# bobwan1995/cliora

Measured on AMD Instinct MI355X. Metric: sentences/sec (inside+outside fwd+bwd), len-20 d=400 bsz=64, higher is better.
Workload: dtype f32 (compose GEMMs: 3x bf16 MFMA per product, fp32 accumulate)

## Files before the change

### cliora_amd/csrc/api_mlp.hip

```cpp
#include "api_mlp_launch.hpp"
#include "ragged_kernels.hpp"
#include "resident_kernels.hpp"
#include "vl_kernels.hpp"

static bool wavefront_pays(const Plan& p, int env) {
    if (p.L <= 2 || env == 0) return false;
    if (env >= 1) return true;
    const double row_floats_per_level = (double)(p.R_in + p.R_out) / (2.0 * (p.L - 1)) * p.Dp;
    return row_floats_per_level >= 100e3;
}

static bool merged_pays(const Plan& p) {
    if (p.arch != 0 || p.L <= 2) return false;
    if (g_cliora_wavefront != 2 && !(g_cliora_wavefront < 0 && wavefront_pays(p, -1))) return false;
    for (size_t e = 0; e < (size_t)2 * p.L; ++e) {
        const int sp = p.level_geom[e * PLEVEL_INTS + 6];
        if (p.level_geom[e * PLEVEL_INTS + 1] > 0 && !project2_parts_ok(sp)) return false;
    }
    return true;
}

static size_t resident_lds_bytes(const Plan& p) {
    return ((size_t)(p.share ? 7 : 8) * p.Dp * p.Dp + (size_t)RES_WAVES * RES_SCR) * sizeof(float);
}
// ... 496 lines not shown
    const float *x_span, *obj_span, *drop_mask, *inside_h, *IS, *outside_h, *OS;
    const float *d_inside_h, *d_inside_s, *d_outside_h, *d_outside_s;
    float *ws, *wb, *d_x_span, *d_obj_span;
    int ran_outside;
    hipStream_t st;

    const Plan& p = plan->p;
    const FwdLayout& f = p.fwd;
    const BwdLayout& bw = p.bwd;
    const Dev dv = dev_views(p);
    const int B = p.B, L = p.L, D = p.D, Dp = p.Dp, C = p.C, nb = p.nblk, ldpi = nb * Dp;
    const bool vl = p.R > 0, padded = D != Dp;
    const bool compress = P && P->root_mat;
    const BwdSchedule schedule = compress ? BwdSchedule::OutsideThenInside
                               : resident_pays(plan, vl, compress) ? BwdSchedule::Resident : BwdSchedule::Wavefront;
    const bool resident = schedule == BwdSchedule::Resident;
    const bool two_streams = schedule == BwdSchedule::Wavefront && ran_outside && wavefront_pays(p, g_cliora_wavefront);
    const hipStream_t sb = two_streams ? plan->side : st, sw = plan->side2;
    const float *IH = padded ? ws + f.ihp : inside_h, *OH = padded ? ws + f.ohp : outside_h;
    const float *X = padded ? ws + f.xp : x_span, *OBJ = vl ? (padded ? ws + f.objp : obj_span) : nullptr;
    const float *IHn = vl ? ws + f.att_u : IH, *nrmIn = vl ? ws + f.att_nrmu : ws + f.nrmi;
    float *VH = wb + bw.vh, *dG = wb + bw.dg, *dStot = wb + bw.dstot, *VHo = wb + bw.vh_o, *dGo = wb + bw.dg_o, *dStoto = wb + bw.dstot_o;
    float *DA = wb + bw.da, *DS = wb + bw.ds, *dPI = wb + bw.dpi, *dPO = wb + bw.dpo, *dU = wb + bw.du;
    float *DZ = wb + bw.dz, *Xp = wb + bw.x, *DPP = wb + bw.dpp, *DPB = wb + bw.dpb;
    const float *Sp = ws + f.sp, *Pp = ws + f.pp, *PI = ws + f.pi;
    const uint32_t* YM = reinterpret_cast<const uint32_t*>(ws + f.ymask);
    const bool fuse_dnorm = schedule == BwdSchedule::Wavefront;
    const int gemm3_shape = split_bf16() ? bwd_gemm3_env() : 0;
    const bool tiled = pair_tiles_ok(Dp) && !resident;
    float *sibPL = p.share ? wb + bw.sib_pl : dPI + (size_t)3 * Dp, *sibQL = p.share ? wb + bw.sib_ql : dPI + (size_t)4 * Dp;
    const int ldsib = p.share ? Dp : ldpi;
    const int sib_split = two_streams ? (L * 2) / 5 : 0;

    bool sibling_runs(int s_level) const { return s_level >= 0 && s_level <= p.L - 1 && ran_outside && s_level < sib_split; }

    template <class EP>
    int project_bwd(hipStream_t s, const float* WT, const float* WTfrag, const float* W3s, int K, int ncell, const LevelRowsA& rows, EP ep) const {
        if (gemm3_shape > 0) return launch_rows_direct3x(s, W3s, K, p.Dp, ncell, rows, ep, gemm3_shape);
        return launch_rows_direct(s, WT, WTfrag, IMG_FRAG_F32, K, p.Dp, ncell, rows, ep);
    }
    int project_bwd_level(hipStream_t s, bool outside, const LevelArgs& g, bool fused_norm) const {
        const int ldp = outside ? Dp : ldpi, ncell = B * g.Lc;
        const float *WT = ws + (outside ? f.w1roT : f.wcatT), *WTfrag = ws + (outside ? f.w1roT3 : f.wcatT3), *W3s = ws + (outside ? f.w1roT3s : f.wcatT3s);
        const LevelRowsA rows{outside ? dPO : dPI, ldp, p.C, g.off, g.Lc};
        float* vh = outside ? VHo : VH;
        if (fused_norm)
            return project_bwd(s, WT, WTfrag, W3s, ldp, ncell, rows,
                               NormBwdLevelE{outside ? dGo : dG, vh, outside ? OH : IH, ws + (outside ? f.nrmo : f.nrmi),
                                             wb + (outside ? bw.dots_o : bw.dots), Dp, p.C, g.off, g.Lc, p.normalize});
        return project_bwd(s, WT, WTfrag, W3s, ldp, ncell, rows, StoreLevelE{vh, Dp, p.C, g.off, g.Lc, nullptr, 1});
    }

    int outside_bwd_step(int level, hipEvent_t done) const {
        const LevelArgs g = level_args(p, level, true);
        const int ncell = B * g.Lc;
        const bool fused_norm = fuse_dnorm && level >= 1 && level <= L - 2;
        hipLaunchKernelGGL(cell_gather_bwd_out, dim3(ncell), dim3(256), 0, sb, g, p.D, d_outside_h,
                           level == L - 1 ? nullptr : d_outside_s, dv.use[ROLE_OUTB], DA, DS, PI, ldpi, p.blk_qlo, dPO, VHo, dStoto,
                           OH, ws + f.po, fused_norm ? wb + bw.dots_o : nullptr);
        LAUNCHOK("cell_gather_bwd_out");
        if (level >= 1) OKR(project_bwd_level(sb, true, g, fused_norm));
        if (level == L - 1) {
            if (compress) {
                hipLaunchKernelGGL(cell_dnorm, dim3(cells_grid(ncell)), dim3(256), 0, sb, g, VHo, OH, ws + f.nrmo, p.normalize, dGo);
                LAUNCHOK("cell_dnorm(root)");
                return CLIORA_OK;
            }
            LAUNCH_SIGNALLING(done, root_bwd, dim3(1), dim3(ROOT_WAVES * 64), 0, sb, B, C, Dp, VHo, OH, ws + f.nrmo, p.normalize, wb + bw.groot);
            LAUNCHOK("root_bwd");
            return CLIORA_OK;
        }
        if (!fused_norm) {
            hipLaunchKernelGGL(cell_dnorm, dim3(cells_grid(ncell)), dim3(256), 0, sb, g, VHo, OH, ws + f.nrmo, p.normalize, dGo);
            LAUNCHOK("cell_dnorm(out)");
        }
        {
            ProfScope ps(CLIORA_KCLASS_COMPOSE_BWD, sb);
            OKR(launch_level_compose_bwd(sb, ws + f.w2oT, ws + f.w2oT3, f.S3, Dp, f.ct3, f.ncb3, pair_level(p, level, true), dGo, YM, Pp,
                                         PI + (size_t)p.blk_plo * Dp, ldpi, ws + f.po, Dp, ws + f.b2o, DA, DZ, Xp, DPP, DPB, tiled));
        }
        const int s_level = L - 2 - level;
        const bool sib_last = sibling_runs(s_level);
        LAUNCH_SIGNALLING(sib_last ? nullptr : done, cell_dsoftmax, dim3(cells_grid(ncell)), dim3(256), 0, sb, g, f.ncb3, DPP, DPB, Sp, Pp, OS, dStoto, DS);
        LAUNCHOK("cell_dsoftmax(out)");
        if (sib_last) {
            const LevelArgs gi = level_args(p, s_level, false);
            LAUNCH_SIGNALLING(done, cell_gather_bwd_sib, dim3(B * gi.Lc), dim3(256), 0, sb, gi, dv.use[ROLE_OUTA], DA, DS, OH, sibPL, sibQL, ldsib, wb + bw.sib_s);
            LAUNCHOK("cell_gather_bwd_sib");
        }
        return CLIORA_OK;
    }

    WgradPlacement wgrad_placement() const {
        static const int ksplit_env = [] { const char* e = getenv("CLIORA_WGRAD_SPLIT_LEVEL"); return e ? atoi(e) : -1; }();
        const bool wcat_split_path = split_bf16() && tn_pairs_strided_ok(p.Dp);
        const bool sw_beside = plan->side2_beside;
        WgradPlacement w{};
        w.ksplit = ksplit_env >= 0 ? ksplit_env : !sw_beside ? 0
                 : wcat_split_path ? std::max(1, std::min(2 * L / 5, L - 1)) : std::min(2, L - 1);
        w.tail_cells = p.C;
        static const int early_env = [] { const char* e = getenv("CLIORA_WGRAD_EARLY_STEP"); return e ? atoi(e) : -2; }();
        const int early_auto = L >= 16 && sw_beside ? L / 2 + 1 : -1;
        const int early_pick = early_env == -2 ? early_auto : early_env;
        w.J_early = (p.share && ran_outside && schedule == BwdSchedule::Wavefront && early_pick >= 0 && early_pick <= L - 3) ? early_pick : -1;
        const int early2_pick = L >= 28 ? (w.J_early + L) / 2 : -1;
        w.J_early2 = (w.J_early >= 0 && early2_pick > w.J_early && early2_pick <= L - 3) ? early2_pick : -1;
        return w;
    }
    int wcat_grad(hipStream_t s_, int off, int hi, int accumulate) const {
        if (tn_pairs_strided_ok(Dp) && (long long)B * hi >= 512 && (long long)B * hi < (1LL << 22)) {
            return launch_tn_level_block(s_, dPI, ldpi, IH, B, C, off, hi, Dp, wb + bw.slab2, bw.slab_floats, wb + bw.gwcat, wb + bw.gbcat, accumulate,
                                         std::max(8, (180 / (3 * nb)) / 4 * 4), nb);
        }
        return launch_tn(s_, B * hi, ldpi, Dp, Dp, LevelRowsA{dPI, ldpi, C, off, hi}, LevelRowsA{IH, Dp, C, off, hi}, wb + bw.slab2,
                         bw.slab_floats, wb + bw.gwcat, wb + bw.gbcat, accumulate);
    }
    int pair_rows_early(WgradPlacement& w, int j) const {
        const bool first = j == w.J_early;
        const bool second = tiled && w.J_early >= 0 && j == w.J_early2;
        if (!first && !second) return CLIORA_OK;
// ... 96 lines not shown
        const size_t DD = (size_t)Dp * Dp;
        if (vl && d_obj_span && padded) add_copy(t, d_obj_span, D, B * p.R, D, wb + bw.dobjp, Dp, B * p.R, D, 0, 0, 0);
        if (G->leaf_w) add_copy(t, G->leaf_w, D, D, D, wb + bw.gwl, Dp, D, D, 0, 0, 0);
        if (G->leaf_b) add_copy(t, G->leaf_b, D, 1, D, wb + bw.gbl, Dp, 1, D, 0, 0, 0);
        if (G->root_h && !compress) add_copy(t, G->root_h, D, 1, D, wb + bw.groot, Dp, 1, D, 0, 0, 0);
        if (G->root_mat && compress) add_copy(t, G->root_mat, D, D, D, wb + bw.groot_mat, Dp, D, D, 0, 0, 1);
        const bool early = p.share && w.J_early >= 0;
        if (G->in_w1) {
            add_copy(t, G->in_w1, 2 * D, D, D, wb + bw.gwcat, Dp, D, D, 0, 0, 0);
            add_copy(t, G->in_w1 + D, 2 * D, D, D, wb + bw.gwcat + DD, Dp, D, D, 0, 0, 0, p.share ? wb + bw.gw1ro : nullptr, Dp, D, D, 0, 0, 0);
        }
        if (G->in_b1) add_copy(t, G->in_b1, D, 1, D, wb + bw.gbcat, Dp, 1, D, 0, 0, 0);
        if (G->in_mat) add_copy(t, G->in_mat, D, D, D, wb + bw.gwcat + 2 * DD, Dp, D, D, 0, 0, 1);
        if (G->in_w2) add_copy(t, G->in_w2, D, D, D, wb + bw.gw2i, Dp, D, D, 0, 0, 0, early ? wb + bw.gw2o : nullptr, Dp, D, D, 0, 0, 0);
        if (G->in_b2) add_copy(t, G->in_b2, D, 1, D, wb + bw.gb2i, Dp, 1, D, 0, 0, 0, early ? wb + bw.gb2o : nullptr, Dp, 1, D, 0, 0, 0);
        if (!p.share) {
            if (G->out_w1) {
                add_copy(t, G->out_w1, 2 * D, D, D, wb + bw.gwcat + 3 * DD, Dp, D, D, 0, 0, 0);
                add_copy(t, G->out_w1 + D, 2 * D, D, D, wb + bw.gw1ro, Dp, D, D, 0, 0, 0);
            }
            if (G->out_b1) add_copy(t, G->out_b1, D, 1, D, wb + bw.gbcat + 3 * Dp, Dp, 1, D, 0, 0, 0);
            if (G->out_mat) add_copy(t, G->out_mat, D, D, D, wb + bw.gwcat + 4 * DD, Dp, D, D, 0, 0, 1);
            if (G->out_w2) add_copy(t, G->out_w2, D, D, D, wb + bw.gw2o, Dp, D, D, 0, 0, 0);
            if (G->out_b2) add_copy(t, G->out_b2, D, 1, D, wb + bw.gb2o, Dp, 1, D, 0, 0, 0);
        }
        return run_copies(st, t);
    }

    int inside_bwd_step(WgradPlacement& w, int level) const {
        hipStream_t sa = st;
        const LevelArgs g = level_args(p, level, false);
        const int ncell = B * g.Lc;
        const bool fused_norm = fuse_dnorm && p.share && !vl && level >= 1 && level <= L - 2;
        hipLaunchKernelGGL(cell_gather_bwd_in, dim3(ncell), dim3(256), 0, sa, g, p.D, d_inside_h,
                           level == 0 ? nullptr : d_inside_s, dv.use[ROLE_INA], dv.use[ROLE_INB], dv.use[ROLE_OUTA],
                           !ran_outside ? 0 : (level < sib_split ? 1 : 2),
                           sibPL, sibQL, ldsib, wb + bw.sib_s, DA, DS, PI, ldpi, p.share, IH, OH, dPI, VH, dStot,
                           ws + f.bcat, fused_norm ? wb + bw.dots : nullptr);
        LAUNCHOK("cell_gather_bwd_in");
        if (level == 0) {
            HIPOK(hipEventRecord(plan->ev_fork[2], sa));
            w.dpi_done_recorded = true;
        }
        if (level <= L - 2) OKR(project_bwd_level(sa, false, g, fused_norm));
        else if (compress && ran_outside)
            OKR(launch_rows_direct(sa, ws + f.rootwT, PROJ_IMG(f.rootwT3), Dp, Dp, ncell, LevelRowsA{dGo, Dp, C, g.off, g.Lc},
                                   StoreLevelE{VH, Dp, C, g.off, g.Lc, nullptr, 1}));
        if (vl) {
            with_regions(p.R, [&](auto NR) {
                hipLaunchKernelGGL(cell_attend_bwd<decltype(NR)::value>, dim3(ncell), dim3(256), 0, sa, g, VH, IH, ws + f.nrmi, p.normalize, OBJ, p.R,
                                   drop_mask, ws + f.att_pk, wb + bw.dctx, wb + bw.pmo, wb + bw.dsc, IHn, nrmIn, level >= 1 ? dG : (float*)nullptr);
            });
            LAUNCHOK("cell_attend_bwd");
        }
        if (level == w.ksplit && level >= 1) {
            HIPOK(hipEventRecord(plan->ev_fork[2], sa));
            HIPOK(hipStreamWaitEvent(sw, plan->ev_fork[2], 0));
            OKR(wcat_grad(sw, g.off, w.tail_cells - g.off, w.tail_cells < C));
            w.tail_cells = g.off;
        }
        if (level == 0) return CLIORA_OK;
        if (!fused_norm && !vl) {
            hipLaunchKernelGGL(cell_dnorm, dim3(cells_grid(ncell)), dim3(256), 0, sa, g, VH, IHn, nrmIn, p.normalize, dG);
            LAUNCHOK("cell_dnorm(in)");
        }
        {
            ProfScope ps(CLIORA_KCLASS_COMPOSE_BWD, sa);
            OKR(launch_level_compose_bwd(sa, ws + f.w2iT, ws + f.w2iT3, f.S3, Dp, f.ct3, f.ncb3, pair_level(p, level, false), dG, YM, Pp, PI, ldpi,
                                         PI + Dp, ldpi, ws + f.b2i, DA, DZ, Xp, DPP, DPB, tiled));
        }
        hipLaunchKernelGGL(cell_dsoftmax, dim3(cells_grid(ncell)), dim3(256), 0, sa, g, f.ncb3, DPP, DPB, Sp, Pp, IS, dStot, DS);
        LAUNCHOK("cell_dsoftmax(in)");
        if (level == 1 && two_streams) HIPOK(hipEventRecord(plan->ev_join[2], sa));
        return CLIORA_OK;
    }

    int backward_wavefront(WgradPlacement& w) const {
        for (int j = 0; j <= L - 1; ++j) {
            if (ran_outside) OKR(outside_bwd_step(j, two_streams ? plan->ev_level[j] : nullptr));
            if (two_streams && j >= 1) HIPOK(hipStreamWaitEvent(st, plan->ev_level[j - 1], 0));
            OKR(inside_bwd_step(w, L - 1 - j));
            OKR(pair_rows_early(w, j));
        }
        return CLIORA_OK;
    }

    int backward_outside_then_inside(WgradPlacement& w) const {
        for (int j = 0; j <= L - 1 && ran_outside; ++j) OKR(outside_bwd_step(j, nullptr));
        for (int j = 0; j <= L - 1; ++j) OKR(inside_bwd_step(w, L - 1 - j));
        if (ran_outside)
            return launch_tn(st, p.B, Dp, Dp, Dp, LevelRowsA{dGo, Dp, C, C - 1, 1}, LevelRowsA{IH, Dp, C, C - 1, 1}, wb + bw.slab, bw.slab_floats,
                             wb + bw.groot_mat, (float*)nullptr);
        HIPOK(hipMemsetAsync(wb + bw.groot_mat, 0, (size_t)Dp * Dp * sizeof(float), st));
        return CLIORA_OK;
    }

    int backward_resident() const {
        ResArgs a = resident_args(plan, ws, const_cast<float*>(IH), const_cast<float*>(OH), const_cast<float*>(IS), const_cast<float*>(OS), ran_outside);
        a.dIH = d_inside_h; a.dIS = d_inside_s; a.dOH = d_outside_h; a.dOS = d_outside_s;
        a.VHo = VHo; a.dPI = dPI; a.dPO = dPO; a.DA = DA; a.DS = DS; a.DZ = DZ; a.Xrows = Xp; a.dU = dU; a.dX = d_x_span;
        a.trace = res_trace() ? reinterpret_cast<unsigned long long*>(plan->trace_words) : nullptr;
        OKR(cliora_ensure_max_lds((const void*)resident_bwd));
        {
            ProfScope ps(CLIORA_KCLASS_COMPOSE_BWD, st);
            hipLaunchKernelGGL(resident_bwd, dim3(std::min(p.B, std::max(1, plan->ncu))), dim3(RES_THREADS), resident_lds_bytes(p), st, a);
// ... 67 lines not shown
```

### cliora_amd/csrc/api_mlp_launch.hpp

```cpp
#pragma once
#include "api_common.hpp"
#include "level_kernels.hpp"

template <class F>
static auto with_regions(int R, F&& f) {
    return R <= 36 ? f(Int<9>{}) : f(Int<16>{});
}

template <class F>
static int with_compose_shape(int ct, int Dp, F&& f) {
    auto mode = [&](auto CT, auto K16) { return split_bf16() ? f(CT, K16, Bool<false>{}) : f(CT, K16, Bool<true>{}); };
    if (ct == 5 && Dp == 400) return mode(Int<5>{}, Int<25>{});
    return with_int<5, 4, 2, 1>(ct, [&](auto CT) { return mode(CT, Int<0>{}); });
}
static int compose_image_stride(int S3, int Dp) { return split_bf16() ? S3 : Dp; }

template <class F>
static int with_parts(int SP, F&& f) {
    return with_int<1, 2, 3, 4>(SP, f);
}
static bool project2_parts_ok(int SP) { return SP == 1 || SP == 2 || SP == 4; }
template <class F>
static int with_parts2(int SP, F&& f) {
    return with_int<1, 2, 4>(SP, f);
// ... 15 lines not shown
        constexpr bool f32 = decltype(F32)::value;
        OKR(cliora_ensure_max_lds((const void*)level_compose_fwd<ct_, k16, f32>));
        hipLaunchKernelGGL((level_compose_fwd<ct_, k16, f32>), dim3(sg.gx, ncb), dim3(512), compose_lds_bytes(ct_, S, true), st, sg.Wimg, S, Dp, sg.lv,
                           sg.PA, sg.lda, sg.PB, sg.ldb, sg.bias, Pp, sg.TG, sg.SP, sg.ntask, sg.HP, hp_stride, Dp, ymask, Y);
        LAUNCHOK("level_compose_fwd");
        return CLIORA_OK;
    });
}

static int launch_level_compose2(hipStream_t st, const ComposeSeg& a, const ComposeSeg& b, int S3, int Dp, int ct, int ncb, const float* Pp,
                                 size_t hp_stride, uint32_t* ymask, float* Y) {
    if (a.gx + b.gx <= 0) return CLIORA_OK;
    const int S = compose_image_stride(S3, Dp);
    const int gx = xcd_pad(a.gx + b.gx);
    return with_compose_shape(ct, Dp, [&](auto CT, auto K16, auto F32) {
        constexpr int ct_ = decltype(CT)::value, k16 = decltype(K16)::value;
        constexpr bool f32 = decltype(F32)::value;
        if constexpr (k16 == 25 && !f32) {
            const size_t lds_dual = compose_lds_bytes(ct_, S, true) + (size_t)ct_ * 16 * sizeof(float);
            OKR(cliora_ensure_max_lds((const void*)level_compose_fwd2<ct_, k16, f32, 2>));
            hipLaunchKernelGGL((level_compose_fwd2<ct_, k16, f32, 2>), dim3(gx, ncb), dim3(512), lds_dual, st, a, b, S, Dp, Pp, hp_stride, Dp, ymask, Y);
            LAUNCHOK("level_compose_fwd2(dual)");
        } else {
            OKR(cliora_ensure_max_lds((const void*)level_compose_fwd2<ct_, k16, f32>));
            hipLaunchKernelGGL((level_compose_fwd2<ct_, k16, f32>), dim3(gx, ncb), dim3(512), compose_lds_bytes(ct_, S, true), st, a, b, S, Dp, Pp, hp_stride, Dp, ymask, Y);
            LAUNCHOK("level_compose_fwd2");
        }
        return CLIORA_OK;
    });
}

static int launch_level_compose_bwd(hipStream_t st, const float* WT, const float* WTimg, int S3, int Dp, int ct, int ncb, const PairLevel& lv,
                                    const float* dG, const uint32_t* ymask, const float* Pp, const float* PA, int lda, const float* PB,
                                    int ldb, const float* b2, float* DA, float* DZ, float* X, float* DPP, float* DPB, bool tiled = false, int cus = 256) {
    if (lv.N <= 0 || lv.ncell <= 0) return CLIORA_OK;
    const uint32_t* I = reinterpret_cast<const uint32_t*>(split_bf16() ? WTimg : WT);
    const int S = compose_image_stride(S3, Dp), K = Dp;
    auto launch = [&](auto CT, auto K16, auto F32, auto TILED) {
        constexpr int ct_ = decltype(CT)::value, k16 = decltype(K16)::value;
        constexpr bool f32 = decltype(F32)::value, tiled_ = decltype(TILED)::value;
        OKR(cliora_ensure_max_lds((const void*)level_compose_bwd<ct_, k16, f32, tiled_>));
        const int gx = ws_grid((lv.ncell + 15) / 16 * lv.N, ncb, 8, cus);
        hipLaunchKernelGGL((level_compose_bwd<ct_, k16, f32, tiled_>), dim3(gx, ncb), dim3(512), compose_lds_bytes(ct_, S, false) + (size_t)((K + 31) / 32 * 32) * sizeof(float), st, I, S, K, lv, dG, ymask,
                           Pp, PA, lda, PB, ldb, b2, K, DA, DZ, X, DPP, DPB);
        LAUNCHOK("level_compose_bwd");
        return CLIORA_OK;
    };
    if (tiled) {
        if (!split_bf16() || ct != 5 || Dp != 400) return fail(CLIORA_EINVAL, "tiled pair-row operands: d = 400 in split-bf16 mode only");
        return launch(Int<5>{}, Int<25>{}, Bool<false>{}, Bool<true>{});
    }
    return with_compose_shape(ct, Dp, [&](auto CT, auto K16, auto F32) { return launch(CT, K16, F32, Bool<false>{}); });
}

static int launch_level_project(hipStream_t st, int SP, const ProjSeg& q, hipEvent_t stop, bool lng) {
    const int nt = q.ntc, nrg = (q.ncell + 15) / 16;
    const int nrgp = xcd_pad(nrg);
    auto launch = [&](auto CT, auto SP_, auto LONG) {
        const int ncb = nt / decltype(CT)::value;
        LAUNCH_SIGNALLING(stop, (level_project<decltype(CT)::value, decltype(SP_)::value, decltype(LONG)::value>), dim3(q.sc.nscore + nrgp * ncb),
                          dim3(256), 0, st, q.Wfrag, q.K, nrg, nrgp, ncb, q.ncell, q.Lc, q.C, q.off, q.HP, q.hp_stride, q.normalize, q.bias, q.P,
                          q.ldp, q.H, q.nrm, q.sc);
        LAUNCHOK("level_project");
        return CLIORA_OK;
    };
    const bool wide = nt % 5 == 0 && nrg * (nt / 5) >= KSPLIT_MIN_BLOCKS;
    return with_long(lng, [&](auto LONG) {
        return with_parts(SP, [&](auto SP_) { return wide ? launch(Int<5>{}, SP_, LONG) : launch(Int<1>{}, SP_, LONG); });
    });
}

static int launch_level_project2(hipStream_t st, int SP0, int SP1, const ProjSeg& a, const ProjSeg& b, bool lng) {
    if (!project2_parts_ok(SP0) || !project2_parts_ok(SP1)) return fail(CLIORA_EINVAL, "level_project2: parts per level must be 1, 2 or 4");
    const int n = a.sc.nscore + b.sc.nscore + a.nproj + b.nproj + a.nfin + b.nfin;
    if (n <= 0) return CLIORA_OK;
    return with_long(lng, [&](auto LONG) {
        return with_parts2(SP0, [&](auto S0) {
// ... 9 lines not shown
```

### cliora_amd/csrc/chart_kernels.hpp

```cpp
#pragma once
#include <hip/hip_runtime.h>
#include <stdint.h>

#include "gemm_kernels.hpp"

namespace cliora {

constexpr float UNIT_EPS = 1e-8f;

__device__ __forceinline__ int cell_of_block(int bid, int B, int Lc) {
    const int n8 = (B >> 3) * 8 * Lc;
    if (bid >= n8) return bid;
    const int x = bid & 7, q = bid >> 3;
    const int bb = q / Lc, p = q - bb * Lc;
    return (bb * 8 + x) * Lc + p;
}

struct LevelArgs {
    int B, C, Dp, Lc, N, off;
    int rowbase;
};

__device__ __forceinline__ float4 ld4(const float* p) { return *reinterpret_cast<const float4*>(p); }
__device__ __forceinline__ void st4(float* p, float4 v) { *reinterpret_cast<float4*>(p) = v; }
// ... 77 lines not shown
            if (a1) v += f4dot(ld4(qa + 4 * (lane + 64)), ld4(hb + 4 * (lane + 64)));
            d[j] = v;
        }
#pragma unroll
        for (int j = 0; j < 4; ++j) {
            const float s = wave_sum(d[j]) + SA[ar[j]] + SB[br[j]];
            if (lane == 0 && n0 + 4 * j < g.N) sh_s[n0 + 4 * j] = s;
        }
    }
    __syncthreads();
    if (wave != 0) return;
    const float my_s = lane < g.N ? sh_s[lane] : -INFINITY;
    const float m = wave_max(my_s);
    const float e = lane < g.N ? expf(my_s - m) : 0.f;
    const float pn = e / wave_sum(e);
    if (lane < g.N) { Sp[row0 + lane] = my_s; Pp[row0 + lane] = pn; }
    const float st = wave_sum(lane < g.N ? pn * my_s : 0.f);
    if (lane == 0) Sout[(size_t)b * g.C + g.off + p] = st;
}



struct UseTab { const int32_t *off, *row, *stride, *partner; };

__device__ __forceinline__ float4 ld_ext(const float* base, int D, int col) {
    float4 v = f4zero();
    if (col + 0 < D) v.x = base[col + 0];
    if (col + 1 < D) v.y = base[col + 1];
    if (col + 2 < D) v.z = base[col + 2];
    if (col + 3 < D) v.w = base[col + 3];
    return v;
}

__device__ __forceinline__ void gather_uses(const UseTab& ut, int c, int b, int bC, int wave, const float* __restrict__ DA,
                                            const float* __restrict__ DS, int Dp, const float* __restrict__ SRC, int ldsrc,
                                            int col0, int col1, bool act0, bool act1,
                                            float4& da0, float4& da1, float4& x0, float4& x1, float& vS) {
    const int beg = ut.off[c], end = ut.off[c + 1];
    for (int u0 = beg + wave; u0 < end; u0 += 16) {
        size_t r[4];
        float ds[4], m[4];
        const float* sp[4];
#pragma unroll
        for (int j = 0; j < 4; ++j) {
            const int uu = min(u0 + 4 * j, end - 1);
            m[j] = (u0 + 4 * j < end) ? 1.f : 0.f;
            r[j] = (size_t)ut.row[uu] + (size_t)b * ut.stride[uu];
            sp[j] = SRC + (size_t)(bC + ut.partner[uu]) * ldsrc;
        }
#pragma unroll
        for (int j = 0; j < 4; ++j) ds[j] = DS[r[j]] * m[j];
        float4 a0[4], a1[4], s0[4], s1[4];
#pragma unroll
        for (int j = 0; j < 4; ++j) {
            a0[j] = act0 ? ld4(DA + r[j] * Dp + col0) : f4zero();
            s0[j] = act0 ? ld4(sp[j] + col0) : f4zero();
            a1[j] = act1 ? ld4(DA + r[j] * Dp + col1) : f4zero();
            s1[j] = act1 ? ld4(sp[j] + col1) : f4zero();
        }
#pragma unroll
        for (int j = 0; j < 4; ++j) {
            vS += ds[j];
            da0 = f4fma(m[j], a0[j], da0);
            da1 = f4fma(m[j], a1[j], da1);
            x0 = f4fma(ds[j], s0[j], x0);
            x1 = f4fma(ds[j], s1[j], x1);
        }
    }
}

constexpr int GATHER_SLOTS = 10;
__device__ __forceinline__ void wg_sum_pairs(float4 (*sh)[GATHER_SLOTS][64], int wave, int lane, int nslots, float4* v) {
    if (wave >= 2)
        for (int k = 0; k < nslots; ++k) sh[wave - 2][k][lane] = v[k];
    __syncthreads();
    if (wave < 2)
        for (int k = 0; k < nslots; ++k) v[k] = f4add(v[k], sh[wave][k][lane]);
    __syncthreads();
    if (wave == 1)
        for (int k = 0; k < nslots; ++k) sh[0][k][lane] = v[k];
    __syncthreads();
    if (wave == 0)
        for (int k = 0; k < nslots; ++k) v[k] = f4add(v[k], sh[0][k][lane]);
}

static __global__ __launch_bounds__(256) void cell_gather_bwd_in(LevelArgs g, int D, const float* __restrict__ dH_ext, const float* __restrict__ dS_ext,
                                                          UseTab ina, UseTab inb, UseTab outa, int with_outside,
                                                          float* __restrict__ sib_pl, float* __restrict__ sib_ql, int ldsib,
                                                          const float* __restrict__ sib_s,
                                                          const float* __restrict__ DA, const float* __restrict__ DS,
                                                          const float* __restrict__ PI, int ldpi, int share,
                                                          const float* __restrict__ IH, const float* __restrict__ OH,
                                                          float* __restrict__ dPI, float* __restrict__ VH, float* __restrict__ dStot,
                                                          const float* __restrict__ bcat, float* __restrict__ dots) {
    __shared__ float4 sh[2][GATHER_SLOTS][64];
    __shared__ float sh_s[4], sh_s2[4];
    const int lane = threadIdx.x & 63, wave = threadIdx.x >> 6;
    const int t = cell_of_block(blockIdx.x, g.B, g.Lc);
    const int b = t / g.Lc, p = t - b * g.Lc;
    const int c = g.off + p;
    const size_t crow = (size_t)b * g.C + c;
    const int Dp = g.Dp, nv = Dp >> 2;
    const int bC = b * g.C;
    const bool act0 = lane < nv, act1 = lane + 64 < nv;
    const int col0 = 4 * lane, col1 = 4 * (lane + 64);
    float vS = 0.f;
    float4 v[GATHER_SLOTS];
#pragma unroll
    for (int k = 0; k < GATHER_SLOTS; ++k) v[k] = f4zero();
    const bool sib = with_outside == 1 && share && wave == 0;
    float4 sp0 = f4zero(), sp1 = f4zero(), sq0 = f4zero(), sq1 = f4zero();
    if (sib && act0) { sp0 = ld4(sib_pl + crow * Dp + col0); sq0 = ld4(sib_ql + crow * Dp + col0); }
    if (sib && act1) { sp1 = ld4(sib_pl + crow * Dp + col1); sq1 = ld4(sib_ql + crow * Dp + col1); }
    const float ss = (with_outside == 1 && wave == 0) ? sib_s[crow] : 0.f;
    gather_uses(inb, c, b, bC, wave, DA, DS, Dp, PI + 2 * Dp, ldpi, col0, col1, act0, act1, v[4], v[5], v[0], v[1], vS);
    gather_uses(ina, c, b, bC, wave, DA, DS, Dp, IH, Dp, col0, col1, act0, act1, v[2], v[3], v[6], v[7], vS);
    wg_sum_pairs(sh, wave, lane, 8, v);
    if (with_outside == 2) {
        float4 w[4] = {f4zero(), f4zero(), f4zero(), f4zero()};
        __syncthreads();
        float vSo = 0.f;
        gather_uses(outa, c, b, bC, wave, DA, DS, Dp, OH, Dp, col0, col1, act0, act1, w[0], w[1], w[2], w[3], vSo);
        wg_sum_pairs(sh, wave, lane, 4, w);
        if (lane == 0) sh_s2[wave] = vSo;
        sp0 = w[0]; sp1 = w[1]; sq0 = w[2]; sq1 = w[3];
        if (!share && wave == 0) {
            if (act0) { st4(sib_pl + crow * ldsib + col0, sp0); st4(sib_ql + crow * ldsib + col0, sq0); }
            if (act1) { st4(sib_pl + crow * ldsib + col1, sp1); st4(sib_ql + crow * ldsib + col1, sq1); }
        }
        if (!share) { sp0 = sp1 = sq0 = sq1 = f4zero(); }
    }
    if (lane == 0) sh_s[wave] = vS;
    __syncthreads();
    if (wave != 0) return;
    const float sso = with_outside == 2 ? ((sh_s2[0] + sh_s2[1]) + sh_s2[2]) + sh_s2[3] : ss;
    const float vs = ((sh_s[0] + sh_s[1]) + sh_s[2]) + sh_s[3] + sso + (dS_ext ? dS_ext[crow] : 0.f);
    float* o = dPI + crow * ldpi;
    if (act0) {
        const float4 e = dH_ext ? ld_ext(dH_ext + crow * D, D, col0) : f4zero();
        st4(o + col0, f4add(v[2], sp0)); st4(o + Dp + col0, v[4]); st4(o + 2 * Dp + col0, f4add(v[6], sq0));
        st4(VH + crow * Dp + col0, f4add(v[0], e));
    }
    if (act1) {
        const float4 e = dH_ext ? ld_ext(dH_ext + crow * D, D, col1) : f4zero();
        st4(o + col1, f4add(v[3], sp1)); st4(o + Dp + col1, v[5]); st4(o + 2 * Dp + col1, f4add(v[7], sq1));
        st4(VH + crow * Dp + col1, f4add(v[1], e));
    }
    if (lane == 0) dStot[crow] = vs;
    if (dots) {
        float d = 0.f;
        const float* hr = IH + crow * Dp;
        const float* pr = PI + crow * ldpi;
        if (act0) {
            const float4 e = dH_ext ? ld_ext(dH_ext + crow * D, D, col0) : f4zero();
            d += f4dot(ld4(hr + col0), f4add(v[0], e));
            const float4 b = ld4(bcat + col0), pl = ld4(pr + col0);
            d += f4dot(f4add(v[2], sp0), make_float4(pl.x - b.x, pl.y - b.y, pl.z - b.z, pl.w - b.w));
            d += f4dot(v[4], ld4(pr + Dp + col0)) + f4dot(f4add(v[6], sq0), ld4(pr + 2 * Dp + col0));
        }
        if (act1) {
            const float4 e = dH_ext ? ld_ext(dH_ext + crow * D, D, col1) : f4zero();
            d += f4dot(ld4(hr + col1), f4add(v[1], e));
            const float4 b = ld4(bcat + col1), pl = ld4(pr + col1);
            d += f4dot(f4add(v[3], sp1), make_float4(pl.x - b.x, pl.y - b.y, pl.z - b.z, pl.w - b.w));
            d += f4dot(v[5], ld4(pr + Dp + col1)) + f4dot(f4add(v[7], sq1), ld4(pr + 2 * Dp + col1));
        }
        d = wave_sum(d);
        if (lane == 0) dots[crow] = d;
    }
}

static __global__ __launch_bounds__(256) void cell_gather_bwd_sib(LevelArgs g, UseTab outa, const float* __restrict__ DA, const float* __restrict__ DS,
                                                           const float* __restrict__ OH, float* __restrict__ out_pl, float* __restrict__ out_ql,
                                                           int ldo, float* __restrict__ sib_s) {
    __shared__ float4 sh[2][GATHER_SLOTS][64];
    __shared__ float sh_s[4];
    const int lane = threadIdx.x & 63, wave = threadIdx.x >> 6;
    const int t = cell_of_block(blockIdx.x, g.B, g.Lc);
    const int b = t / g.Lc, p = t - b * g.Lc;
    const int c = g.off + p;
    const size_t crow = (size_t)b * g.C + c;
    const int Dp = g.Dp, nv = Dp >> 2;
    const int bC = b * g.C;
    const bool act0 = lane < nv, act1 = lane + 64 < nv;
    const int col0 = 4 * lane, col1 = 4 * (lane + 64);
    float vS = 0.f;
    float4 v[GATHER_SLOTS];
#pragma unroll
    for (int k = 0; k < 4; ++k) v[k] = f4zero();
    gather_uses(outa, c, b, bC, wave, DA, DS, Dp, OH, Dp, col0, col1, act0, act1, v[2], v[3], v[0], v[1], vS);
    wg_sum_pairs(sh, wave, lane, 4, v);
    if (lane == 0) sh_s[wave] = vS;
    __syncthreads();
    if (wave != 0) return;
    if (act0) { st4(out_pl + crow * ldo + col0, v[2]); st4(out_ql + crow * ldo + col0, v[0]); }
    if (act1) { st4(out_pl + crow * ldo + col1, v[3]); st4(out_ql + crow * ldo + col1, v[1]); }
    if (lane == 0) sib_s[crow] = ((sh_s[0] + sh_s[1]) + sh_s[2]) + sh_s[3];
}

static __global__ __launch_bounds__(256) void cell_gather_bwd_out(LevelArgs g, int D, const float* __restrict__ dH_ext, const float* __restrict__ dS_ext,
                                                           UseTab outb, const float* __restrict__ DA, const float* __restrict__ DS,
                                                           const float* __restrict__ PI, int ldpi, int blk_qlo,
                                                           float* __restrict__ dPO, float* __restrict__ VH, float* __restrict__ dStot,
                                                           const float* __restrict__ OHc, const float* __restrict__ PO, float* __restrict__ dots) {
    __shared__ float4 sh[2][GATHER_SLOTS][64];
    __shared__ float sh_s[4];
    const int lane = threadIdx.x & 63, wave = threadIdx.x >> 6;
    const int t = cell_of_block(blockIdx.x, g.B, g.Lc);
    const int b = t / g.Lc, p = t - b * g.Lc;
    const int c = g.off + p;
    const size_t crow = (size_t)b * g.C + c;
    const int Dp = g.Dp, nv = Dp >> 2;
    const int bC = b * g.C;
    const bool act0 = lane < nv, act1 = lane + 64 < nv;
    const int col0 = 4 * lane, col1 = 4 * (lane + 64);
    float vS = 0.f;
    float4 v[GATHER_SLOTS];
#pragma unroll
    for (int k = 0; k < 4; ++k) v[k] = f4zero();
    gather_uses(outb, c, b, bC, wave, DA, DS, Dp, PI + (size_t)blk_qlo * Dp, ldpi, col0, col1, act0, act1, v[2], v[3], v[0], v[1], vS);
    wg_sum_pairs(sh, wave, lane, 4, v);
    if (lane == 0) sh_s[wave] = vS;
    __syncthreads();
    if (wave != 0) return;
    const float vs = ((sh_s[0] + sh_s[1]) + sh_s[2]) + sh_s[3] + (dS_ext ? dS_ext[crow] : 0.f);
    if (act0) {
        const float4 e = dH_ext ? ld_ext(dH_ext + crow * D, D, col0) : f4zero();
        st4(dPO + crow * Dp + col0, v[2]); st4(VH + crow * Dp + col0, f4add(v[0], e));
    }
    if (act1) {
        const float4 e = dH_ext ? ld_ext(dH_ext + crow * D, D, col1) : f4zero();
        st4(dPO + crow * Dp + col1, v[3]); st4(VH + crow * Dp + col1, f4add(v[1], e));
    }
    if (lane == 0) dStot[crow] = vs;
    if (dots) {
        float d = 0.f;
        if (act0) {
            const float4 e = dH_ext ? ld_ext(dH_ext + crow * D, D, col0) : f4zero();
            d += f4dot(ld4(OHc + crow * Dp + col0), f4add(v[0], e)) + f4dot(v[2], ld4(PO + crow * Dp + col0));
        }
        if (act1) {
            const float4 e = dH_ext ? ld_ext(dH_ext + crow * D, D, col1) : f4zero();
            d += f4dot(ld4(OHc + crow * Dp + col1), f4add(v[1], e)) + f4dot(v[3], ld4(PO + crow * Dp + col1));
        }
        d = wave_sum(d);
        if (lane == 0) dots[crow] = d;
    }
}

__device__ __forceinline__ void unit_norm_bwd(float4& v0, float4& v1, float4 h0, float4 h1, float nr, int normalize) {
    if (!normalize) return;
    if (nr > UNIT_EPS) {
        const float dot = wave_sum(f4dot(v0, h0) + f4dot(v1, h1));
// ... 152 lines not shown
```

### cliora_amd/csrc/level_kernels.hpp

```cpp
#pragma once
#include <hip/hip_runtime.h>
#include <stdint.h>

#include "chart_kernels.hpp"
#include "wgrad_tiles.hpp"

namespace cliora {

struct PairLevel {
    const int32_t *pa, *pb;
    int Lc, N, C, ncell;
    int rowbase;
    int off;
    long long tilebase;
};

constexpr int LC_SLOTS = 4;

struct StepOperand { u32x4 h, l; };
template <bool F32>
__device__ __forceinline__ StepOperand make_operand(int psrc, const float4& f0, const float4& f1) {
    const float4 a0 = to_mfma_lanes(psrc, f0), a1 = to_mfma_lanes(psrc, f1);
    StepOperand o;
    if constexpr (F32) {
// ... 1081 lines not shown
                                        x.z > 0.f ? pn * u.z : 0.f, x.w > 0.f ? pn * u.w : 0.f));
                if (!TILED) st4(X + o, x);
            }
            if (TILED)
                store_split_tile(reinterpret_cast<uint32_t*>(X) + ((size_t)(lv.tilebase + tile) * NT + by * CT + c) * 256 + 2 * lane,
                                 ok ? x : f4zero());
        }
        dp += __shfl_xor(dp, 1);
        dp += __shfl_xor(dp, 2);
        if (ok && lg == 0) DPP[prow * gy + by] = dp;
        if (!has_next) break;
        ctx = ctxn;
        tile = ntile;
    }
}

static __global__ __launch_bounds__(256) void cell_dnorm(LevelArgs g, const float* __restrict__ VH, const float* __restrict__ H,
                                                         const float* __restrict__ nrm, int normalize, float* __restrict__ dG) {
    const int lane = threadIdx.x & 63;
    const int t = blockIdx.x * 4 + (threadIdx.x >> 6);
    if (t >= g.B * g.Lc) return;
    const int b = t / g.Lc, p = t - b * g.Lc;
    const size_t crow = (size_t)b * g.C + g.off + p;
    const int Dp = g.Dp, nv = Dp >> 2;
    const bool a0 = lane < nv, a1 = lane + 64 < nv;
    float4 v0 = f4zero(), v1 = f4zero(), h0 = f4zero(), h1 = f4zero();
    if (a0) { v0 = ld4(VH + crow * Dp + 4 * lane); h0 = ld4(H + crow * Dp + 4 * lane); }
    if (a1) { v1 = ld4(VH + crow * Dp + 4 * (lane + 64)); h1 = ld4(H + crow * Dp + 4 * (lane + 64)); }
    unit_norm_bwd(v0, v1, h0, h1, nrm[crow], normalize);
    if (a0) st4(dG + crow * Dp + 4 * lane, v0);
    if (a1) st4(dG + crow * Dp + 4 * (lane + 64), v1);
}

static __global__ __launch_bounds__(256) void cell_dsoftmax(LevelArgs g, int ncb, const float* __restrict__ DPP, const float* __restrict__ DPB,
                                                            const float* __restrict__ Sp, const float* __restrict__ Pp,
                                                            const float* __restrict__ Schart, const float* __restrict__ dStot,
                                                            float* __restrict__ DS) {
    const int lane = threadIdx.x & 63;
    const int t = blockIdx.x * 4 + (threadIdx.x >> 6);
    if (t >= g.B * g.Lc || g.N == 0) return;
    const int b = t / g.Lc, p = t - b * g.Lc;
    const size_t crow = (size_t)b * g.C + g.off + p;
    const size_t row0 = (size_t)g.rowbase + (size_t)t * g.N;
    const bool an = lane < g.N;
    float dp = an ? DPB[row0 + lane] : 0.f;
    if (an)
        for (int cb = 0; cb < ncb; ++cb) dp += DPP[(row0 + lane) * ncb + cb];
    const float pn = an ? Pp[row0 + lane] : 0.f;
    const float sn = an ? Sp[row0 + lane] : 0.f;
    const float mean = wave_sum(pn * dp);
    const float ds = pn * ((dp - mean) + dStot[crow] * (1.f + (sn - Schart[crow])));
    if (an) DS[row0 + lane] = ds;
}

}
```

Before: 21730.

## Fold per-level dsoftmax into the next gather kernel as extra blocks and inline recompute

In the wavefront backward schedule, the standalone cell_dsoftmax launch after each compose level is removed. Its work now runs as extra trailing blocks of the next level's gather kernel, and gathers that read fresh DS rows recompute the softmax gradient inline via wave shuffle instead of loading it. The completion event moves onto the compose_bwd launch. This cuts one launch and one dependency step per level on both the inside and outside chains, but it adds redundant recomputation, more register pressure in gather_uses, and a possible race between the ride blocks that write DS and the gather blocks that read it.

```diff
diff --git a/cliora_amd/csrc/api_mlp.hip b/cliora_amd/csrc/api_mlp.hip
--- a/cliora_amd/csrc/api_mlp.hip
+++ b/cliora_amd/csrc/api_mlp.hip
@@ -552,6 +552,23 @@
     const int ldsib = p.share ? Dp : ldpi;
     const int sib_split = two_streams ? (L * 2) / 5 : 0;
 
+    const bool ds_rides = schedule == BwdSchedule::Wavefront;
+    DsLevel ds_level(int level, bool outside, bool on = true) const {
+        DsLevel q{};
+        if (!on || !ds_rides || level < 0 || level > L - 1 || (outside && !ran_outside)) return q;
+        q.g = level_args(p, level, outside);
+        q.ncb = f.ncb3; q.DPP = DPP; q.DPB = DPB; q.Sp = Sp; q.Pp = Pp;
+        q.Schart = outside ? OS : IS; q.dStot = outside ? dStoto : dStot;
+        return q;
+    }
+    static int ride_blocks(const DsLevel& q) { return q.g.N > 0 ? (int)cells_grid(q.g.B * q.g.Lc) : 0; }
+    int dsoftmax_alone(hipStream_t s, int level, bool outside, hipEvent_t done) const {
+        DsLevel q{level_args(p, level, outside), f.ncb3, DPP, DPB, Sp, Pp, outside ? OS : IS, outside ? dStoto : dStot};
+        LAUNCH_SIGNALLING(done, cell_dsoftmax, dim3(cells_grid(q.g.B * q.g.Lc)), dim3(256), 0, s, q, DS);
+        LAUNCHOK("cell_dsoftmax");
+        return CLIORA_OK;
+    }
+
     bool sibling_runs(int s_level) const { return s_level >= 0 && s_level <= p.L - 1 && ran_outside && s_level < sib_split; }
 
     template <class EP>
@@ -575,8 +592,9 @@
         const LevelArgs g = level_args(p, level, true);
         const int ncell = B * g.Lc;
         const bool fused_norm = fuse_dnorm && level >= 1 && level <= L - 2;
-        hipLaunchKernelGGL(cell_gather_bwd_out, dim3(ncell), dim3(256), 0, sb, g, p.D, d_outside_h,
-                           level == L - 1 ? nullptr : d_outside_s, dv.use[ROLE_OUTB], DA, DS, PI, ldpi, p.blk_qlo, dPO, VHo, dStoto,
+        const DsLevel nwo = ds_level(level - 1, true);
+        hipLaunchKernelGGL(cell_gather_bwd_out, dim3(ncell + ride_blocks(nwo)), dim3(256), 0, sb, g, p.D, d_outside_h,
+                           level == L - 1 ? nullptr : d_outside_s, dv.use[ROLE_OUTB], DA, DS, nwo, ncell, PI, ldpi, p.blk_qlo, dPO, VHo, dStoto,
                            OH, ws + f.po, fused_norm ? wb + bw.dots_o : nullptr);
         LAUNCHOK("cell_gather_bwd_out");
         if (level >= 1) OKR(project_bwd_level(sb, true, g, fused_norm));
@@ -594,18 +612,18 @@
             hipLaunchKernelGGL(cell_dnorm, dim3(cells_grid(ncell)), dim3(256), 0, sb, g, VHo, OH, ws + f.nrmo, p.normalize, dGo);
             LAUNCHOK("cell_dnorm(out)");
         }
+        const int s_level = L - 2 - level;
+        const bool sib_last = sibling_runs(s_level);
         {
             ProfScope ps(CLIORA_KCLASS_COMPOSE_BWD, sb);
             OKR(launch_level_compose_bwd(sb, ws + f.w2oT, ws + f.w2oT3, f.S3, Dp, f.ct3, f.ncb3, pair_level(p, level, true), dGo, YM, Pp,
-                                         PI + (size_t)p.blk_plo * Dp, ldpi, ws + f.po, Dp, ws + f.b2o, DA, DZ, Xp, DPP, DPB, tiled));
-        }
-        const int s_level = L - 2 - level;
-        const bool sib_last = sibling_runs(s_level);
-        LAUNCH_SIGNALLING(sib_last ? nullptr : done, cell_dsoftmax, dim3(cells_grid(ncell)), dim3(256), 0, sb, g, f.ncb3, DPP, DPB, Sp, Pp, OS, dStoto, DS);
-        LAUNCHOK("cell_dsoftmax(out)");
+                                         PI + (size_t)p.blk_plo * Dp, ldpi, ws + f.po, Dp, ws + f.b2o, DA, DZ, Xp, DPP, DPB, tiled, 256,
+                                         ds_rides && !sib_last ? done : nullptr));
+        }
+        if (!ds_rides) OKR(dsoftmax_alone(sb, level, true, sib_last ? nullptr : done));
         if (sib_last) {
             const LevelArgs gi = level_args(p, s_level, false);
-            LAUNCH_SIGNALLING(done, cell_gather_bwd_sib, dim3(B * gi.Lc), dim3(256), 0, sb, gi, dv.use[ROLE_OUTA], DA, DS, OH, sibPL, sibQL, ldsib, wb + bw.sib_s);
+            LAUNCH_SIGNALLING(done, cell_gather_bwd_sib, dim3(B * gi.Lc), dim3(256), 0, sb, gi, dv.use[ROLE_OUTA], DA, DS, ds_level(level, true), OH, sibPL, sibQL, ldsib, wb + bw.sib_s);
             LAUNCHOK("cell_gather_bwd_sib");
         }
         return CLIORA_OK;
@@ -768,10 +786,11 @@
         const LevelArgs g = level_args(p, level, false);
         const int ncell = B * g.Lc;
         const bool fused_norm = fuse_dnorm && p.share && !vl && level >= 1 && level <= L - 2;
-        hipLaunchKernelGGL(cell_gather_bwd_in, dim3(ncell), dim3(256), 0, sa, g, p.D, d_inside_h,
-                           level == 0 ? nullptr : d_inside_s, dv.use[ROLE_INA], dv.use[ROLE_INB], dv.use[ROLE_OUTA],
-                           !ran_outside ? 0 : (level < sib_split ? 1 : 2),
-                           sibPL, sibQL, ldsib, wb + bw.sib_s, DA, DS, PI, ldpi, p.share, IH, OH, dPI, VH, dStot,
+        const int with_outside = !ran_outside ? 0 : (level < sib_split ? 1 : 2);
+        const DsLevel nwi = ds_level(level + 1, false), nwo = ds_level(L - 2 - level, true, with_outside == 2);
+        hipLaunchKernelGGL(cell_gather_bwd_in, dim3(ncell + ride_blocks(nwi)), dim3(256), 0, sa, g, p.D, d_inside_h,
+                           level == 0 ? nullptr : d_inside_s, dv.use[ROLE_INA], dv.use[ROLE_INB], dv.use[ROLE_OUTA], with_outside,
+                           sibPL, sibQL, ldsib, wb + bw.sib_s, DA, DS, nwi, nwo, ncell, PI, ldpi, p.share, IH, OH, dPI, VH, dStot,
                            ws + f.bcat, fused_norm ? wb + bw.dots : nullptr);
         LAUNCHOK("cell_gather_bwd_in");
         if (level == 0) {
@@ -805,8 +824,7 @@
             OKR(launch_level_compose_bwd(sa, ws + f.w2iT, ws + f.w2iT3, f.S3, Dp, f.ct3, f.ncb3, pair_level(p, level, false), dG, YM, Pp, PI, ldpi,
                                          PI + Dp, ldpi, ws + f.b2i, DA, DZ, Xp, DPP, DPB, tiled));
         }
-        hipLaunchKernelGGL(cell_dsoftmax, dim3(cells_grid(ncell)), dim3(256), 0, sa, g, f.ncb3, DPP, DPB, Sp, Pp, IS, dStot, DS);
-        LAUNCHOK("cell_dsoftmax(in)");
+        if (!ds_rides) OKR(dsoftmax_alone(sa, level, false, nullptr));
         if (level == 1 && two_streams) HIPOK(hipEventRecord(plan->ev_join[2], sa));
         return CLIORA_OK;
     }
diff --git a/cliora_amd/csrc/api_mlp_launch.hpp b/cliora_amd/csrc/api_mlp_launch.hpp
--- a/cliora_amd/csrc/api_mlp_launch.hpp
+++ b/cliora_amd/csrc/api_mlp_launch.hpp
@@ -71,8 +71,12 @@
 
 static int launch_level_compose_bwd(hipStream_t st, const float* WT, const float* WTimg, int S3, int Dp, int ct, int ncb, const PairLevel& lv,
                                     const float* dG, const uint32_t* ymask, const float* Pp, const float* PA, int lda, const float* PB,
-                                    int ldb, const float* b2, float* DA, float* DZ, float* X, float* DPP, float* DPB, bool tiled = false, int cus = 256) {
-    if (lv.N <= 0 || lv.ncell <= 0) return CLIORA_OK;
+                                    int ldb, const float* b2, float* DA, float* DZ, float* X, float* DPP, float* DPB, bool tiled = false, int cus = 256,
+                                    hipEvent_t stop = nullptr) {
+    if (lv.N <= 0 || lv.ncell <= 0) {
+        if (stop) HIPOK(hipEventRecord(stop, st));
+        return CLIORA_OK;
+    }
     const uint32_t* I = reinterpret_cast<const uint32_t*>(split_bf16() ? WTimg : WT);
     const int S = compose_image_stride(S3, Dp), K = Dp;
     auto launch = [&](auto CT, auto K16, auto F32, auto TILED) {
@@ -80,8 +84,8 @@
         constexpr bool f32 = decltype(F32)::value, tiled_ = decltype(TILED)::value;
         OKR(cliora_ensure_max_lds((const void*)level_compose_bwd<ct_, k16, f32, tiled_>));
         const int gx = ws_grid((lv.ncell + 15) / 16 * lv.N, ncb, 8, cus);
-        hipLaunchKernelGGL((level_compose_bwd<ct_, k16, f32, tiled_>), dim3(gx, ncb), dim3(512), compose_lds_bytes(ct_, S, false) + (size_t)((K + 31) / 32 * 32) * sizeof(float), st, I, S, K, lv, dG, ymask,
-                           Pp, PA, lda, PB, ldb, b2, K, DA, DZ, X, DPP, DPB);
+        LAUNCH_SIGNALLING(stop, (level_compose_bwd<ct_, k16, f32, tiled_>), dim3(gx, ncb), dim3(512), compose_lds_bytes(ct_, S, false) + (size_t)((K + 31) / 32 * 32) * sizeof(float), st, I, S, K, lv, dG, ymask,
+                          Pp, PA, lda, PB, ldb, b2, K, DA, DZ, X, DPP, DPB);
         LAUNCHOK("level_compose_bwd");
         return CLIORA_OK;
     };
diff --git a/cliora_amd/csrc/chart_kernels.hpp b/cliora_amd/csrc/chart_kernels.hpp
--- a/cliora_amd/csrc/chart_kernels.hpp
+++ b/cliora_amd/csrc/chart_kernels.hpp
@@ -133,24 +133,91 @@
     return v;
 }
 
+struct DsLevel {
+    LevelArgs g;
+    int ncb;
+    const float *DPP, *DPB, *Sp, *Pp;
+    const float *Schart, *dStot;
+};
+constexpr int DS_CB = 8;
+struct DsTerms { float dpb, part[DS_CB], pn, sn, dst, sc; const float* pp; bool an; };
+__device__ __forceinline__ DsTerms cell_ds_load(const DsLevel& q, size_t row0, size_t crow, int lane, bool on) {
+    DsTerms o;
+    o.an = on && lane < q.g.N;
+    o.dpb = o.pn = o.sn = o.dst = o.sc = 0.f;
+#pragma unroll
+    for (int cb = 0; cb < DS_CB; ++cb) o.part[cb] = 0.f;
+    const size_t row = row0 + min(lane, q.g.N - 1);
+    o.pp = q.DPP + row * q.ncb;
+    if (on) {
+        o.dpb = q.DPB[row];
+#pragma unroll
+        for (int cb = 0; cb < DS_CB; ++cb)
+            if (cb < q.ncb) o.part[cb] = o.pp[cb];
+        o.pn = q.Pp[row];
+        o.sn = q.Sp[row];
+        o.dst = q.dStot[crow];
+        o.sc = q.Schart[crow];
+    }
+    return o;
+}
+__device__ __forceinline__ float cell_ds_finish(const DsLevel& q, const DsTerms& o) {
+    float dp = o.dpb;
+#pragma unroll
+    for (int cb = 0; cb < DS_CB; ++cb)
+        if (cb < q.ncb) dp += o.part[cb];
+    if (o.an)
+        for (int cb = DS_CB; cb < q.ncb; ++cb) dp += o.pp[cb];
+    dp = o.an ? dp : 0.f;
+    const float pn = o.an ? o.pn : 0.f, sn = o.an ? o.sn : 0.f;
+    const float mean = wave_sum(pn * dp);
+    return pn * ((dp - mean) + o.dst * (1.f + (sn - o.sc)));
+}
+__device__ __forceinline__ void ds_ride_block(const DsLevel& q, int blk, float* __restrict__ DS) {
+    const int lane = threadIdx.x & 63;
+    const int t = blk * 4 + (threadIdx.x >> 6);
+    if (t >= q.g.B * q.g.Lc || q.g.N == 0) return;
+    const int b = t / q.g.Lc, p = t - b * q.g.Lc;
+    const size_t row0 = (size_t)q.g.rowbase + (size_t)t * q.g.N;
+    const float ds = cell_ds_finish(q, cell_ds_load(q, row0, (size_t)b * q.g.C + q.g.off + p, lane, true));
+    if (lane < q.g.N) DS[row0 + lane] = ds;
+}
+
 __device__ __forceinline__ void gather_uses(const UseTab& ut, int c, int b, int bC, int wave, const float* __restrict__ DA,
-                                            const float* __restrict__ DS, int Dp, const float* __restrict__ SRC, int ldsrc,
+                                            const float* __restrict__ DS, const DsLevel& nw, int Dp, const float* __restrict__ SRC, int ldsrc,
                                             int col0, int col1, bool act0, bool act1,
                                             float4& da0, float4& da1, float4& x0, float4& x1, float& vS) {
     const int beg = ut.off[c], end = ut.off[c + 1];
+    const int lane = threadIdx.x & 63;
+    const int nwN = max(nw.g.N, 1);
+    const unsigned nw_rows = (unsigned)(nw.g.Lc * nw.g.N);
     for (int u0 = beg + wave; u0 < end; u0 += 16) {
         size_t r[4];
         float ds[4], m[4];
         const float* sp[4];
+        int q0[4];
 #pragma unroll
         for (int j = 0; j < 4; ++j) {
             const int uu = min(u0 + 4 * j, end - 1);
             m[j] = (u0 + 4 * j < end) ? 1.f : 0.f;
-            r[j] = (size_t)ut.row[uu] + (size_t)b * ut.stride[uu];
+            const int row = ut.row[uu];
+            q0[j] = row - nw.g.rowbase;
+            r[j] = (size_t)row + (size_t)b * ut.stride[uu];
             sp[j] = SRC + (size_t)(bC + ut.partner[uu]) * ldsrc;
         }
-#pragma unroll
-        for (int j = 0; j < 4; ++j) ds[j] = DS[r[j]] * m[j];
+        DsTerms nt[4];
+        bool fresh[4];
+        int nsplit[4];
+#pragma unroll
+        for (int j = 0; j < 4; ++j) {
+            const int q0s = __builtin_amdgcn_readfirstlane(q0[j]);
+            fresh[j] = (unsigned)q0s < nw_rows;
+            const int p = fresh[j] ? q0s / nwN : 0;
+            nsplit[j] = fresh[j] ? q0s - p * nwN : 0;
+            nt[j] = cell_ds_load(nw, (size_t)nw.g.rowbase + (size_t)(b * nw.g.Lc + p) * nwN, (size_t)bC + nw.g.off + p, lane, fresh[j]);
+            ds[j] = 0.f;
+            if (!fresh[j]) ds[j] = DS[r[j]];
+        }
         float4 a0[4], a1[4], s0[4], s1[4];
 #pragma unroll
         for (int j = 0; j < 4; ++j) {
@@ -158,6 +225,11 @@
             s0[j] = act0 ? ld4(sp[j] + col0) : f4zero();
             a1[j] = act1 ? ld4(DA + r[j] * Dp + col1) : f4zero();
             s1[j] = act1 ? ld4(sp[j] + col1) : f4zero();
+        }
+#pragma unroll
+        for (int j = 0; j < 4; ++j) {
+            const float dn = __shfl(cell_ds_finish(nw, nt[j]), nsplit[j]);
+            ds[j] = (fresh[j] ? dn : ds[j]) * m[j];
         }
 #pragma unroll
         for (int j = 0; j < 4; ++j) {
@@ -189,13 +261,14 @@
                                                           UseTab ina, UseTab inb, UseTab outa, int with_outside,
                                                           float* __restrict__ sib_pl, float* __restrict__ sib_ql, int ldsib,
                                                           const float* __restrict__ sib_s,
-                                                          const float* __restrict__ DA, const float* __restrict__ DS,
+                                                          const float* __restrict__ DA, float* DS, DsLevel nwi, DsLevel nwo, int ngather,
                                                           const float* __restrict__ PI, int ldpi, int share,
                                                           const float* __restrict__ IH, const float* __restrict__ OH,
                                                           float* __restrict__ dPI, float* __restrict__ VH, float* __restrict__ dStot,
                                                           const float* __restrict__ bcat, float* __restrict__ dots) {
     __shared__ float4 sh[2][GATHER_SLOTS][64];
     __shared__ float sh_s[4], sh_s2[4];
+    if ((int)blockIdx.x >= ngather) { ds_ride_block(nwi, (int)blockIdx.x - ngather, DS); return; }
     const int lane = threadIdx.x & 63, wave = threadIdx.x >> 6;
     const int t = cell_of_block(blockIdx.x, g.B, g.Lc);
     const int b = t / g.Lc, p = t - b * g.Lc;
@@ -214,14 +287,14 @@
     if (sib && act0) { sp0 = ld4(sib_pl + crow * Dp + col0); sq0 = ld4(sib_ql + crow * Dp + col0); }
     if (sib && act1) { sp1 = ld4(sib_pl + crow * Dp + col1); sq1 = ld4(sib_ql + crow * Dp + col1); }
     const float ss = (with_outside == 1 && wave == 0) ? sib_s[crow] : 0.f;
-    gather_uses(inb, c, b, bC, wave, DA, DS, Dp, PI + 2 * Dp, ldpi, col0, col1, act0, act1, v[4], v[5], v[0], v[1], vS);
-    gather_uses(ina, c, b, bC, wave, DA, DS, Dp, IH, Dp, col0, col1, act0, act1, v[2], v[3], v[6], v[7], vS);
+    gather_uses(inb, c, b, bC, wave, DA, DS, nwi, Dp, PI + 2 * Dp, ldpi, col0, col1, act0, act1, v[4], v[5], v[0], v[1], vS);
+    gather_uses(ina, c, b, bC, wave, DA, DS, nwi, Dp, IH, Dp, col0, col1, act0, act1, v[2], v[3], v[6], v[7], vS);
     wg_sum_pairs(sh, wave, lane, 8, v);
     if (with_outside == 2) {
         float4 w[4] = {f4zero(), f4zero(), f4zero(), f4zero()};
         __syncthreads();
         float vSo = 0.f;
-        gather_uses(outa, c, b, bC, wave, DA, DS, Dp, OH, Dp, col0, col1, act0, act1, w[0], w[1], w[2], w[3], vSo);
+        gather_uses(outa, c, b, bC, wave, DA, DS, nwo, Dp, OH, Dp, col0, col1, act0, act1, w[0], w[1], w[2], w[3], vSo);
         wg_sum_pairs(sh, wave, lane, 4, w);
         if (lane == 0) sh_s2[wave] = vSo;
         sp0 = w[0]; sp1 = w[1]; sq0 = w[2]; sq1 = w[3];
@@ -271,7 +344,7 @@
     }
 }
 
-static __global__ __launch_bounds__(256) void cell_gather_bwd_sib(LevelArgs g, UseTab outa, const float* __restrict__ DA, const float* __restrict__ DS,
+static __global__ __launch_bounds__(256) void cell_gather_bwd_sib(LevelArgs g, UseTab outa, const float* __restrict__ DA, const float* __restrict__ DS, DsLevel nwo,
                                                            const float* __restrict__ OH, float* __restrict__ out_pl, float* __restrict__ out_ql,
                                                            int ldo, float* __restrict__ sib_s) {
     __shared__ float4 sh[2][GATHER_SLOTS][64];
@@ -289,7 +362,7 @@
     float4 v[GATHER_SLOTS];
 #pragma unroll
     for (int k = 0; k < 4; ++k) v[k] = f4zero();
-    gather_uses(outa, c, b, bC, wave, DA, DS, Dp, OH, Dp, col0, col1, act0, act1, v[2], v[3], v[0], v[1], vS);
+    gather_uses(outa, c, b, bC, wave, DA, DS, nwo, Dp, OH, Dp, col0, col1, act0, act1, v[2], v[3], v[0], v[1], vS);
     wg_sum_pairs(sh, wave, lane, 4, v);
     if (lane == 0) sh_s[wave] = vS;
     __syncthreads();
@@ -300,12 +373,13 @@
 }
 
 static __global__ __launch_bounds__(256) void cell_gather_bwd_out(LevelArgs g, int D, const float* __restrict__ dH_ext, const float* __restrict__ dS_ext,
-                                                           UseTab outb, const float* __restrict__ DA, const float* __restrict__ DS,
+                                                           UseTab outb, const float* __restrict__ DA, float* DS, DsLevel nwo, int ngather,
                                                            const float* __restrict__ PI, int ldpi, int blk_qlo,
                                                            float* __restrict__ dPO, float* __restrict__ VH, float* __restrict__ dStot,
                                                            const float* __restrict__ OHc, const float* __restrict__ PO, float* __restrict__ dots) {
     __shared__ float4 sh[2][GATHER_SLOTS][64];
     __shared__ float sh_s[4];
+    if ((int)blockIdx.x >= ngather) { ds_ride_block(nwo, (int)blockIdx.x - ngather, DS); return; }
     const int lane = threadIdx.x & 63, wave = threadIdx.x >> 6;
     const int t = cell_of_block(blockIdx.x, g.B, g.Lc);
     const int b = t / g.Lc, p = t - b * g.Lc;
@@ -319,7 +393,7 @@
     float4 v[GATHER_SLOTS];
 #pragma unroll
     for (int k = 0; k < 4; ++k) v[k] = f4zero();
-    gather_uses(outb, c, b, bC, wave, DA, DS, Dp, PI + (size_t)blk_qlo * Dp, ldpi, col0, col1, act0, act1, v[2], v[3], v[0], v[1], vS);
+    gather_uses(outb, c, b, bC, wave, DA, DS, nwo, Dp, PI + (size_t)blk_qlo * Dp, ldpi, col0, col1, act0, act1, v[2], v[3], v[0], v[1], vS);
     wg_sum_pairs(sh, wave, lane, 4, v);
     if (lane == 0) sh_s[wave] = vS;
     __syncthreads();
diff --git a/cliora_amd/csrc/level_kernels.hpp b/cliora_amd/csrc/level_kernels.hpp
--- a/cliora_amd/csrc/level_kernels.hpp
+++ b/cliora_amd/csrc/level_kernels.hpp
@@ -1137,25 +1137,6 @@
     if (a1) st4(dG + crow * Dp + 4 * (lane + 64), v1);
 }
 
-static __global__ __launch_bounds__(256) void cell_dsoftmax(LevelArgs g, int ncb, const float* __restrict__ DPP, const float* __restrict__ DPB,
-                                                            const float* __restrict__ Sp, const float* __restrict__ Pp,
-                                                            const float* __restrict__ Schart, const float* __restrict__ dStot,
-                                                            float* __restrict__ DS) {
-    const int lane = threadIdx.x & 63;
-    const int t = blockIdx.x * 4 + (threadIdx.x >> 6);
-    if (t >= g.B * g.Lc || g.N == 0) return;
-    const int b = t / g.Lc, p = t - b * g.Lc;
-    const size_t crow = (size_t)b * g.C + g.off + p;
-    const size_t row0 = (size_t)g.rowbase + (size_t)t * g.N;
-    const bool an = lane < g.N;
-    float dp = an ? DPB[row0 + lane] : 0.f;
-    if (an)
-        for (int cb = 0; cb < ncb; ++cb) dp += DPP[(row0 + lane) * ncb + cb];
-    const float pn = an ? Pp[row0 + lane] : 0.f;
-    const float sn = an ? Sp[row0 + lane] : 0.f;
-    const float mean = wave_sum(pn * dp);
-    const float ds = pn * ((dp - mean) + dStot[crow] * (1.f + (sn - Schart[crow])));
-    if (an) DS[row0 + lane] = ds;
-}
-
-}
+static __global__ __launch_bounds__(256) void cell_dsoftmax(DsLevel q, float* __restrict__ DS) { ds_ride_block(q, blockIdx.x, DS); }
+
+}
```

Result: slower. 20550 (-5.4%).
